# mclarsen/cuZFP

Measured on AMD Instinct MI355X. Metric: GB/s input encoded+decoded (device-resident), 3D f32 fixed-rate; % HBM peak, higher is better.
Workload: dtype f32; 1 GPU; 3d_float32_256^3_rate8; maxbits=512, parallelism=z-slab x1, stream_bytes_per_gpu=16777216

## Files before the change

cuzfp_amd/build.py:

```python
from __future__ import annotations

import os
import subprocess
import sys
from concurrent.futures import ThreadPoolExecutor

HERE = os.path.dirname(os.path.abspath(__file__))
ROOT = os.path.dirname(HERE)
CSRC = os.path.join(HERE, "csrc")
LIB = os.path.join(HERE, "lib")
BIN = os.path.join(HERE, "bin")
CLI = os.path.join(HERE, "cli")
OBJ = os.path.join(ROOT, "build", "obj")
INC = os.path.join(ROOT, "include")

ARCH = os.environ.get("CUZFP_OFFLOAD_ARCH", "gfx950")
HIPCC = os.environ.get("HIPCC", "/opt/rocm/bin/hipcc")
CXXFLAGS = ["-O3", "-std=c++17", "-fPIC", f"--offload-arch={ARCH}", f"-I{INC}",
            "-Wall", "-Wno-unused-function", "-Wno-pass-failed"]

KERNEL_UNITS = ["inst_f32", "inst_f64", "inst_i32", "inst_i64",
                "region_f32", "region_f64", "region_i32", "region_i64",
                "update_f32", "update_f64", "update_i32", "update_i64", "truncate",
                "variable_f32", "variable_f64", "region_variable_f32", "region_variable_f64", "truncate_variable",
                "region_variable_coarse_f32", "region_variable_coarse_f64",
                "region_variable_update_f32", "region_variable_update_f64",
                "region_variable_crop_f32", "region_variable_crop_f64",
                "capi"]
HEADERS = ["zfp_block.hpp", "kernels.hpp", "launch.hpp", "wave_index.hpp", "region.hpp", "region_kernels.hpp",
           "region_update_kernels.hpp", "rerate.hpp", "variable_kernels.hpp", "variable_index.hpp",
           "region_variable_kernels.hpp", "rerate_variable.hpp", "source_window.hpp", "variable_coarse.hpp",
           "region_variable_coarse_kernels.hpp", "region_variable_update_kernels.hpp",
           "region_variable_crop_kernels.hpp"]


def _newer(target: str, deps: list[str]) -> bool:
    if not os.path.exists(target):
        return True
    t = os.path.getmtime(target)
    return any(os.path.getmtime(d) > t for d in deps)


def _run(cmd: list[str]) -> None:
    r = subprocess.run(cmd, capture_output=True, text=True)
    if r.returncode != 0:
        sys.stderr.write(r.stdout + r.stderr)
        raise RuntimeError("build failed: " + " ".join(cmd))


def build(verbose: bool = False, jobs: int | None = None) -> dict:
    os.makedirs(LIB, exist_ok=True)
    os.makedirs(OBJ, exist_ok=True)
    hdrs = [os.path.join(CSRC, h) for h in HEADERS] + [os.path.join(INC, "cuzfp_hip.h")]
    jobs_list = []
    objs = []
    for u in KERNEL_UNITS:
        src = os.path.join(CSRC, u + ".hip")
        obj = os.path.join(OBJ, u + ".o")
        objs.append(obj)
        if _newer(obj, [src] + hdrs):
            jobs_list.append([HIPCC, *CXXFLAGS, "-c", src, "-o", obj])
    with ThreadPoolExecutor(max_workers=jobs or min(8, os.cpu_count() or 4)) as ex:
        for cmd in jobs_list:
            if verbose:
                print(" ".join(cmd))
        list(ex.map(_run, jobs_list))
    hip_so = os.path.join(LIB, "libcuzfp_hip.so")
    if jobs_list or _newer(hip_so, objs):
        _run([HIPCC, f"--offload-arch={ARCH}", "-shared", "-fPIC", "-o", hip_so, *objs])
    cpp_src = os.path.join(CSRC, "cuZFP.cpp")
    cpp_so = os.path.join(LIB, "libcuZFP.so")
    if _newer(cpp_so, [cpp_src, hip_so, os.path.join(INC, "cuZFP.h"),
                       os.path.join(INC, "zfp_structs.h")]):
        _run([HIPCC, "-O2", "-std=c++17", "-fPIC", "-shared", f"-I{INC}", "-o", cpp_so, cpp_src,
# ... 16 lines not shown
```

cuzfp_amd/csrc/kernels.hpp:

```cpp
#pragma once
#include <hip/hip_runtime.h>
#include <stdlib.h>

#include <atomic>
#include <type_traits>

#if defined(CUZFP_PROBE) && CUZFP_PROBE == 9
#define CUZFP_STAMP_WAVES 65536
__device__ uint64_t g_stamps[CUZFP_STAMP_WAVES * 10];
__device__ __forceinline__ uint32_t stamp_wave() { return blockIdx.x * (blockDim.x >> 6) + (threadIdx.x >> 6); }
#define ZFP_STAMP(i)                                                              \
  do {                                                                            \
    if ((threadIdx.x & 63) == 0 && stamp_wave() < CUZFP_STAMP_WAVES)              \
      g_stamps[stamp_wave() * 10 + 1 + (i)] = __builtin_amdgcn_s_memtime();      \
  } while (0)
__device__ __forceinline__ void stamp_hwid() {
  uint32_t hw, xcc;
  asm volatile("s_getreg_b32 %0, hwreg(HW_REG_HW_ID)" : "=s"(hw));
  asm volatile("s_getreg_b32 %0, hwreg(HW_REG_XCC_ID)" : "=s"(xcc));
  if ((threadIdx.x & 63) == 0 && stamp_wave() < CUZFP_STAMP_WAVES)
    g_stamps[stamp_wave() * 10] = (uint64_t)hw | ((uint64_t)xcc << 32);
}
__device__ __forceinline__ void stamp_real(int slot) {
  if ((threadIdx.x & 63) == 0 && stamp_wave() < CUZFP_STAMP_WAVES)
// ... 545 lines not shown
  asm volatile("s_waitcnt lgkmcnt(0)" ::: "memory");
  __builtin_amdgcn_wave_barrier();
}

template <int ROWS>
__device__ __forceinline__ void scatter_f64_staged(double* __restrict__ data, const Geometry& g, BlockPos bp,
                                                   const double* f, bool coded, uint64_t* wave_lds,
                                                   uint32_t lane) {
  static_assert(16 % ROWS == 0, "rows a pass");
  uint4* stage = (uint4*)wave_lds;
  double* base = data + ((size_t)(4 * bp.iz) * g.ny + 4 * bp.iy) * g.nx + 4 * (bp.ix - lane);
#pragma unroll
  for (int r0 = 0; r0 < 16; r0 += ROWS) {
    if (coded) {
#pragma unroll
      for (int j = 0; j < ROWS; j++) {
        uint4 a, b;
        __builtin_memcpy(&a, f + 4 * (r0 + j), 16);
        __builtin_memcpy(&b, f + 4 * (r0 + j) + 2, 16);
        stage[j * 128 + 2 * lane] = a;
        stage[j * 128 + 2 * lane + 1] = b;
      }
    } else {
#pragma unroll
      for (int j = 0; j < ROWS; j++) {
        stage[j * 128 + 2 * lane] = uint4{0, 0, 0, 0};
        stage[j * 128 + 2 * lane + 1] = uint4{0, 0, 0, 0};
      }
    }
    wave_lds_sync();
#pragma unroll
    for (int j = 0; j < ROWS; j++) {
      const int r = r0 + j, z = r >> 2, y = r & 3;
      double* row = base + ((size_t)z * g.ny + y) * g.nx;
      st16<true>(row + 2 * lane, stage[j * 128 + lane]);
      st16<true>(row + 128 + 2 * lane, stage[j * 128 + 64 + lane]);
    }
    if (r0 + ROWS < 16) wave_lds_sync();
  }
}

#ifndef CUZFP_F64_ENC_WAVES
#define CUZFP_F64_ENC_WAVES 2
#endif
#ifndef CUZFP_F64_DEC_WAVES
#define CUZFP_F64_DEC_WAVES 2
#endif
#ifndef CUZFP_F32_DEC_WAVES
#define CUZFP_F32_DEC_WAVES 4
#endif
#ifndef CUZFP_F32_ENC_WAVES
#define CUZFP_F32_ENC_WAVES 4
#endif
template <typename Scalar, int DIMS, bool ENC = false> struct occupancy {
  static constexpr int value = (sizeof(Scalar) == 8 && DIMS == 3) ? (ENC ? CUZFP_F64_ENC_WAVES : CUZFP_F64_DEC_WAVES)
                               : (sizeof(Scalar) == 4 && DIMS == 3) ? (ENC ? CUZFP_F32_ENC_WAVES : CUZFP_F32_DEC_WAVES)
                                                                    : 4;
};

template <typename Scalar, int DIMS, bool FAST, bool ALIGNED, bool PRIO = true, int REG = 0, int WPG = kEncWaves>
__device__ __forceinline__ void zfp_encode_body(const Scalar* __restrict__ data, const Geometry& g,
                                                uint64_t* __restrict__ stream, uint32_t bid,
                                                uint32_t* stab, uint32_t* ptab) {
  extern __shared__ __attribute__((aligned(16))) uint64_t lds_all[];
  constexpr int N = 1 << (2 * DIMS);
  const uint32_t wig = wave_in_group();
  const uint32_t wave = g.wave0 + bid * (blockDim.x >> 6) + wig;
  const uint32_t lane = threadIdx.x & 63;
  const uint32_t b = wave * kLanes + lane;
  const bool live_wave = wave < g.wave_end;
  uint64_t* lds = lds_all + (size_t)wig * g.lds_words;
  constexpr bool kGroupSpread = DIMS == 1 || REG != 0;
  if constexpr (DIMS == 2 && REG != 0) {
    for (uint32_t i = threadIdx.x; i < kSpreadTabBytes / 16; i += blockDim.x)
      ((uint4*)stab)[i] = ((const uint4*)g_spread_tab.e)[i];
    __syncthreads();
  }
  if constexpr (DIMS == 1) {
    if (threadIdx.x < 4) ((uint4*)stab)[threadIdx.x] = ((const uint4*)g_spread_tab.e)[threadIdx.x];
    for (uint32_t i = threadIdx.x; i < sizeof(Pair1dLut) / 16; i += blockDim.x)
      ((uint4*)ptab)[i] = ((const uint4*)g_pair1d_lut.e)[i];
    __syncthreads();
  }
  lds_spread* p1d = (lds_spread*)ptab;
  if (!live_wave) return;
  constexpr uint32_t kTabPieces = kSpreadTabBytes / 16;
  uint4 tab16[kTabPieces / kLanes];
  if constexpr (!kGroupSpread) {
#pragma unroll
    for (uint32_t i = 0; i < kTabPieces / kLanes; i++) tab16[i] = ((const uint4*)g_spread_tab.e)[lane + i * kLanes];
  }
  if constexpr (PRIO) __builtin_amdgcn_s_setprio(3);
  lds_spread* lut = (lds_spread*)stab;
  ZFP_STAMP_HWID();
  ZFP_STAMP_REAL(8);
  ZFP_STAMP(0);
  if constexpr (!ALIGNED) {
    for (uint32_t j = lane; j < g.maxbits + 2; j += kLanes) lds[j] = 0;
  }
  const uint32_t W = g.maxbits >> 6;
  Scalar f[N];
  if ((wave + 1) * kLanes <= g.nblocks) {
    gather<Scalar, DIMS, FAST>(data, g, block_pos<DIMS>(g, b), f);
  } else if (b < g.nblocks) {
    gather<Scalar, DIMS, FAST>(data, g, block_pos<DIMS>(g, b), f);
  } else if constexpr (ALIGNED && !REG) {
#pragma unroll
    for (int i = 0; i < N; i++) f[i] = (Scalar)0;
  }
  if constexpr (!kGroupSpread) {
#pragma unroll
    for (uint32_t i = 0; i < kTabPieces / kLanes; i++) ((uint4*)stab)[lane + i * kLanes] = tab16[i];
  }
  if constexpr (REG) {
    wave_lds_sync();
    uint64_t bits = 0;
    if (b < g.nblocks) {
      reg_writer<Scalar, PRIO, REG> wr{lut, p1d, 0, 0};
      if constexpr (REG == 2 || traits<Scalar>::is_int) wr.mb = g.maxbits;
      encode_block<Scalar, DIMS>(f, g.maxbits, wr);
      bits = wr.bits();
    }
    if constexpr (PRIO) __builtin_amdgcn_s_setprio(3);
    if constexpr (REG == 2) {
      if (b < g.nblocks) stream[b] = bits;
    } else {
      if (b < g.nblocks + (g.nblocks & 1u)) ((uint32_t*)stream)[b] = (uint32_t)bits;
    }
    return;
  }
  if constexpr (ALIGNED) {
    uint64_t* mine = lds + lane;
    for (uint32_t j = 0; j < W + kSlackWords; j++) mine[j * 64] = 0;
    if (g.wave0 + (bid + 1) * (blockDim.x >> 6) <= g.wave_end) {
      asm volatile("s_waitcnt vmcnt(0)" ::: "memory");
      __syncthreads();
    }
    wave_lds_sync();
    LdsOrWriter<PRIO> wr{mine, lut, 0, 64 * W, p1d, uniform_const64(0x7fffu)};
    encode_block<Scalar, DIMS>(f, g.maxbits, wr);
  } else if (b < g.nblocks) {
    {
      wave_lds_sync();
      LdsBitWriter<PRIO> wr{lds, lut, lane * g.maxbits, (lane + 1) * g.maxbits, 0, 0, p1d, uniform_const64(0x7fffu)};
      encode_block<Scalar, DIMS>(f, g.maxbits, wr);
    }
  }
  if constexpr (PRIO) __builtin_amdgcn_s_setprio(3);
  wave_lds_sync();
  const uint32_t nb = min((uint32_t)kLanes, g.nblocks - wave * kLanes);
  const uint32_t nwords = (nb * g.maxbits + 63) >> 6;
  uint64_t* out = stream + (size_t)wave * g.maxbits;
  if constexpr (ALIGNED) {
    if (nb == kLanes && g.vec_io && !(W & 1)) {
      uint32_t s, j, ds, dj;
      udivmod_uniform(2 * lane, W, s, j);
      udivmod_uniform(128u, W, ds, dj);
      for (uint32_t k = 2 * lane; k < kLanes * W; k += 128) {
        uint4 v;
        const uint64_t a0 = lds[j * 64 + s], a1 = lds[(j + 1) * 64 + s];
        __builtin_memcpy(&v.x, &a0, 8);
        __builtin_memcpy(&v.z, &a1, 8);
        st16<true>(&out[k], v);
        j += dj;
        s += ds;
        if (j >= W) { j -= W; s++; }
      }
      ZFP_STAMP(6);
      ZFP_STAMP_REAL(9);
      return;
    }
  }
  if constexpr (ALIGNED) {
    if (b < g.nblocks) {
      const uint64_t* mine = lds + lane;
      uint64_t* dst = out + (size_t)lane * W;
      if (g.vec_io && !(W & 1)) {
        for (uint32_t j = 0; j < W; j += 2) {
          uint4 v;
          const uint64_t a0 = mine[j * 64], a1 = mine[(j + 1) * 64];
          __builtin_memcpy(&v.x, &a0, 8);
          __builtin_memcpy(&v.z, &a1, 8);
          st16<kNtStream>(&dst[j], v);
        }
      } else {
        for (uint32_t j = 0; j < W; j++) dst[j] = mine[j * 64];
      }
    }
  } else if (g.vec_io) {
    const uint32_t npairs = nwords >> 1;
    for (uint32_t j = lane; j < npairs; j += kLanes)
      ((uint4*)out)[j] = ((const uint4*)lds)[j];
    if ((nwords & 1) && lane == 0) out[nwords - 1] = lds[nwords - 1];
  } else {
    for (uint32_t j = lane; j < nwords; j += kLanes) out[j] = lds[j];
  }
  ZFP_STAMP(6);
  ZFP_STAMP_REAL(9);
}

template <typename Scalar, int DIMS, bool FAST, bool ALIGNED, bool PRIO = true, int REG = 0, int WPG = kEncWaves>
__global__ __launch_bounds__(kLanes * WPG, (occupancy<Scalar, DIMS, true>::value)) void zfp_encode(const Scalar* __restrict__ data,
                                                                      Geometry g,
                                                                      uint64_t* __restrict__ stream) {
  __shared__ __attribute__((aligned(16))) uint32_t stab[512];
  __shared__ __attribute__((aligned(16))) uint32_t ptab[DIMS == 1 ? 1024 : 4];
  zfp_encode_body<Scalar, DIMS, FAST, ALIGNED, PRIO, REG, WPG>(data, g, stream, blockIdx.x, stab, ptab);
}

template <typename Scalar, int DIMS, bool FAST, bool PRIO = true, int REG = 0, int WPG = kDecWaves>
__device__ __forceinline__ void zfp_decode_body(const uint64_t* __restrict__ stream, const Geometry& g,
                                                Scalar* __restrict__ data, uint32_t bid,
                                                uint32_t* ctab, uint16_t* dtab) {
  extern __shared__ __attribute__((aligned(16))) uint64_t lds_all[];
  constexpr int N = 1 << (2 * DIMS);
  const uint32_t wig = wave_in_group();
  uint32_t wave;
  if constexpr (DIMS == 3 && !REG)
    wave = g.wave0 + decode_wave_of(bid, wig, blockDim.x >> 6, kEncWaves, g.xcd_remap != 0);
  else
    wave = g.wave0 + bid * (blockDim.x >> 6) + wig;
  const uint32_t lane = threadIdx.x & 63;
  const uint32_t b = wave * kLanes + lane;
  const bool live = wave < g.wave_end && b < g.nblocks;
  uint64_t* lds = lds_all + (size_t)wig * g.lds_words;
  uint32_t* lut = ctab;
  auto copy_dtab = [&]() {
    if constexpr (DIMS == 1)
      for (uint32_t i = threadIdx.x; i < sizeof(Plane1dDecLut) / 16; i += blockDim.x)
        ((uint4*)dtab)[i] = ((const uint4*)g_plane1d_lut.e)[i];
  };
  constexpr uint32_t kLutEnd = DIMS == 1 ? kLutPairs * 4 / 16 : sizeof(ChunkLut) / 16;
  const uint32_t* seg = (const uint32_t*)(stream + (size_t)wave * g.maxbits);
  uint32_t* L = (uint32_t*)lds + lane;
  uint64_t blk = 0;
  if constexpr (REG == 32) {
    if (live) blk = seg[lane];
    for (uint32_t i = threadIdx.x; i < kLutEnd; i += blockDim.x)
      ((uint4*)lut)[i] = ((const uint4*)g_chunk_lut.e)[i];
    copy_dtab();
  } else if constexpr (REG) {
    if (live) {
      const uint32_t nb = min((uint32_t)kLanes, g.nblocks - wave * kLanes);
      const uint32_t lim = ((nb * g.maxbits + 63) >> 6) * 2;
      const uint32_t s0 = lane * g.maxbits, d0 = s0 >> 5;
      const uint32_t a0 = seg[d0];
      const uint32_t a1 = d0 + 1 < lim ? seg[d0 + 1] : 0u;
      const uint32_t a2 = d0 + 2 < lim ? seg[d0 + 2] : 0u;
      blk = ((uint64_t)__builtin_amdgcn_alignbit(a1, a0, s0) |
             ((uint64_t)__builtin_amdgcn_alignbit(a2, a1, s0) << 32)) & lowmask(g.maxbits);
    }
    for (uint32_t i = threadIdx.x; i < kLutEnd; i += blockDim.x)
      ((uint4*)lut)[i] = ((const uint4*)g_chunk_lut.e)[i];
    copy_dtab();
  } else {
    const uint32_t D = (g.maxbits + 31) >> 5;
    const bool vec = (g.maxbits & 127) == 0 && g.vec_io;
    constexpr uint32_t kHeld = 8;
    uint4 held[kHeld];
    const bool cont = vec && wave < g.wave_end && g.nblocks - wave * kLanes >= kLanes && D <= 4 * kHeld;
    if (cont) {
      const uint4* src = (const uint4*)seg + lane;
#pragma unroll
      for (uint32_t q = 0; q < kHeld; q++)
        if (4 * q < D) held[q] = ld16<true>(&src[64 * q]);
    } else if (live && vec) {
      const uint4* src = (const uint4*)(seg + lane * D);
#pragma unroll
      for (uint32_t q = 0; q < kHeld; q++)
        if (4 * q < D) held[q] = ld16<kNtStream>(&src[q]);
    }
    for (uint32_t i = threadIdx.x; i < kLutEnd; i += blockDim.x)
      ((uint4*)lut)[i] = ((const uint4*)g_chunk_lut.e)[i];
    copy_dtab();
    if (cont) {
      uint32_t* L0 = (uint32_t*)lds;
      uint32_t sb, j, dsb, dj;
      udivmod_uniform(4 * lane, D, sb, j);
      udivmod_uniform(256u, D, dsb, dj);
#pragma unroll
      for (uint32_t q = 0; q < kHeld; q++)
        if (4 * q < D) {
          L0[(j) * 64 + sb] = held[q].x;
          L0[(j + 1) * 64 + sb] = held[q].y;
          L0[(j + 2) * 64 + sb] = held[q].z;
          L0[(j + 3) * 64 + sb] = held[q].w;
          j += dj;
          sb += dsb;
          if (j >= D) { j -= D; sb++; }
        }
    } else if (live) {
      if (vec) {
#pragma unroll
        for (uint32_t q = 0; q < kHeld; q++)
          if (4 * q < D) {
            L[(4 * q) * 64] = held[q].x;
            L[(4 * q + 1) * 64] = held[q].y;
            L[(4 * q + 2) * 64] = held[q].z;
            L[(4 * q + 3) * 64] = held[q].w;
          }
        const uint4* src = (const uint4*)(seg + lane * D);
        for (uint32_t q = 4 * kHeld; q < D; q += 4) {
          const uint4 v = src[q >> 2];
          L[q * 64] = v.x;
          L[(q + 1) * 64] = v.y;
          L[(q + 2) * 64] = v.z;
          L[(q + 3) * 64] = v.w;
        }
      } else {
        const uint32_t nb = min((uint32_t)kLanes, g.nblocks - wave * kLanes);
        const uint32_t lim = ((nb * g.maxbits + 63) >> 6) * 2;
        const uint32_t s0 = lane * g.maxbits, d0 = s0 >> 5;
        uint32_t prev = seg[d0];
        for (uint32_t j = 0; j < D; j++) {
          const uint32_t nxt = d0 + j + 1 < lim ? seg[d0 + j + 1] : 0u;
          L[j * 64] = __builtin_amdgcn_alignbit(nxt, prev, s0);
          prev = nxt;
        }
        if (g.maxbits & 31) L[(D - 1) * 64] &= (1u << (g.maxbits & 31)) - 1u;
      }
    } else if (wave < g.wave_end) {
      for (uint32_t j = 0; j < D; j++) L[j * 64] = 0;
    }
    if (wave < g.wave_end)
      for (uint32_t j = D; j < D + 5; j++) L[j * 64] = 0;
  }
  __syncthreads();
  if (wave >= g.wave_end) return;
  if constexpr (PRIO) __builtin_amdgcn_s_setprio(3);
  ZFP_STAMP_HWID();
  ZFP_STAMP_REAL(8);
  ZFP_STAMP(0);
  wave_lds_sync();
  ZFP_STAMP(5);
  {
    Scalar f[N];
    bool coded;
    if constexpr (REG) {
      RegReader<PRIO, REG == 32> rd;
      rd.lds32 = L;
      rd.lut32 = lut;
      rd.d1d = dtab;
      rd.set_block(blk);
      rd.init(0);
      coded = decode_block<Scalar, DIMS>(f, g.maxbits, rd);
    } else {
      LdsReader<PRIO> rd;
      rd.lds32 = L;
      rd.lut32 = lut;
      rd.d1d = dtab;
      rd.init(0);
      coded = decode_block<Scalar, DIMS>(f, g.maxbits, rd);
    }
    if constexpr (PRIO) __builtin_amdgcn_s_setprio(3);
    if constexpr (sizeof(Scalar) == 8 && DIMS == 3 && FAST && !REG) {
      if (g.row_stage) {
        const BlockPos bp = block_pos<DIMS>(g, b);
        if (g.row_stage == 4)
          scatter_f64_staged<4>((double*)data, g, bp, (const double*)f, coded, lds, lane);
        else if (g.row_stage == 2)
          scatter_f64_staged<2>((double*)data, g, bp, (const double*)f, coded, lds, lane);
        else
          scatter_f64_staged<1>((double*)data, g, bp, (const double*)f, coded, lds, lane);
        ZFP_STAMP(6);
        ZFP_STAMP_REAL(9);
        return;
      }
    }
    if (b < g.nblocks) {
      if (coded) {
        scatter<Scalar, DIMS, FAST>(data, g, block_pos<DIMS>(g, b), f);
      } else {
        Scalar z[N];
#pragma unroll
        for (int i = 0; i < N; i++) z[i] = (Scalar)0;
        scatter<Scalar, DIMS, FAST>(data, g, block_pos<DIMS>(g, b), z);
      }
    }
  }
  ZFP_STAMP(6);
  ZFP_STAMP_REAL(9);
}

template <typename Scalar, int DIMS, bool FAST, bool PRIO = true, int REG = 0, int WPG = kDecWaves>
__global__ __launch_bounds__(kLanes * WPG, (occupancy<Scalar, DIMS>::value)) void zfp_decode(const uint64_t* __restrict__ stream,
                                                                      Geometry g,
                                                                      Scalar* __restrict__ data) {
  __shared__ __attribute__((aligned(16))) uint32_t ctab[chunk_lut_bytes<DIMS>() / 4];
  __shared__ __attribute__((aligned(16))) uint16_t dtab[DIMS == 1 ? sizeof(Plane1dDecLut) / 2 : 8];
  zfp_decode_body<Scalar, DIMS, FAST, PRIO, REG, WPG>(stream, g, data, blockIdx.x, ctab, dtab);
}

template <typename Scalar, int DIMS, bool PRIO, int REG, int WPG, int K>
__global__ __launch_bounds__(kLanes * WPG, (occupancy<Scalar, DIMS, true>::value)) void zfp_encode_regk(
    const Scalar* __restrict__ data, Geometry g, uint64_t* __restrict__ stream) {
  static_assert(DIMS <= 2 && (REG == 1 || REG == 2) && K >= 2 && K <= 8, "register-writer batches: 1D/2D");
  constexpr int N = 1 << (2 * DIMS);
  __shared__ __attribute__((aligned(16))) uint32_t stab[512];
  __shared__ __attribute__((aligned(16))) uint32_t ptab[DIMS == 1 ? 1024 : 4];
  const uint32_t wig = wave_in_group();
  const uint32_t lane = threadIdx.x & 63;
  const uint32_t w0 = g.wave0 + (blockIdx.x * WPG + wig) * K;
  Scalar f[K][N];
#pragma unroll
  for (int k = 0; k < K; k++) {
    const uint32_t b = (w0 + k) * kLanes + lane;
    if (w0 + k < g.wave_end && b < g.nblocks) gather<Scalar, DIMS, true>(data, g, block_pos<DIMS>(g, b), f[k]);
  }
  if constexpr (DIMS == 2) {
    for (uint32_t i = threadIdx.x; i < kSpreadTabBytes / 16; i += blockDim.x)
      ((uint4*)stab)[i] = ((const uint4*)g_spread_tab.e)[i];
  } else {
    if (threadIdx.x < 4) ((uint4*)stab)[threadIdx.x] = ((const uint4*)g_spread_tab.e)[threadIdx.x];
    for (uint32_t i = threadIdx.x; i < sizeof(Pair1dLut) / 16; i += blockDim.x)
      ((uint4*)ptab)[i] = ((const uint4*)g_pair1d_lut.e)[i];
  }
  __syncthreads();
  lds_spread* lut = (lds_spread*)stab;
  lds_spread* p1d = (lds_spread*)ptab;
#pragma unroll
  for (int k = 0; k < K; k++) {
    const uint32_t b = (w0 + k) * kLanes + lane;
    if (w0 + k >= g.wave_end) break;
    uint64_t bits = 0;
    if (b < g.nblocks) {
      if constexpr (PRIO) __builtin_amdgcn_s_setprio(3);
      reg_writer<Scalar, PRIO, REG> wr{lut, p1d, 0, 0};
      if constexpr (REG == 2 || traits<Scalar>::is_int) wr.mb = g.maxbits;
      encode_block<Scalar, DIMS>(f[k], g.maxbits, wr);
      bits = wr.bits();
    }
    if constexpr (REG == 2) {
      if (b < g.nblocks) stream[b] = bits;
    } else {
      if (b < g.nblocks + (g.nblocks & 1u)) ((uint32_t*)stream)[b] = (uint32_t)bits;
    }
  }
}

__device__ __forceinline__ uint64_t reg_block(const uint64_t* stream, const Geometry& g, uint32_t wave,
                                              uint32_t lane) {
  const uint32_t* seg = (const uint32_t*)(stream + (size_t)wave * g.maxbits);
  const uint32_t nb = min((uint32_t)kLanes, g.nblocks - wave * kLanes);
// ... 63 lines not shown
  static const long forced = [] {
    const char* e = getenv("CUZFP_LDS_CAP_BYTES");
    return (e && *e) ? atol(e) : 0L;
  }();
  if (forced > 0) return (size_t)forced;
  static std::atomic<int> cap[kMaxDevices];
  int dev = 0;
  if (hipGetDevice(&dev) != hipSuccess || dev < 0 || dev >= kMaxDevices) return 65536;
  int c = cap[dev].load(std::memory_order_relaxed);
  if (!c) {
    int n = 0;
    if (hipDeviceGetAttribute(&n, hipDeviceAttributeMaxSharedMemoryPerBlock, dev) != hipSuccess || n <= 0)
      n = 65536;
    cap[dev].store(n, std::memory_order_relaxed);
    c = n;
  }
  return (size_t)c;
}

static inline uint32_t waves_per_group(uint32_t lds_words, size_t shared_bytes, uint32_t most) {
  const size_t cap = lds_cap_bytes();
  uint32_t w = most;
  while (w > 1 && (size_t)w * lds_words * 8 + shared_bytes > cap) w >>= 1;
  return w;
}

static inline bool within_rounds(uint32_t nwaves, int waves_per_simd, uint32_t rounds) {
  static std::atomic<int> cus[kMaxDevices];
  int dev = 0, c = 256;
  if (hipGetDevice(&dev) == hipSuccess && dev >= 0 && dev < kMaxDevices) {
    c = cus[dev].load(std::memory_order_relaxed);
    if (!c) {
      int n = 0;
      if (hipDeviceGetAttribute(&n, hipDeviceAttributeMultiprocessorCount, dev) != hipSuccess || n <= 0) n = 256;
      cus[dev].store(n, std::memory_order_relaxed);
      c = n;
    }
  }
  return nwaves <= (uint32_t)c * 4u * (uint32_t)waves_per_simd * rounds;
}
static inline bool use_priority(uint32_t nwaves, int waves_per_simd, uint32_t rounds) {
  static const int forced = [] {
    const char* e = getenv("CUZFP_PRIO");
    return (e && *e) ? (atoi(e) != 0 ? 1 : 0) : -1;
  }();
  if (forced >= 0) return forced != 0;
  return within_rounds(nwaves, waves_per_simd, rounds);
}

#if defined(CUZFP_XVAR)
constexpr bool kFastOnly = true;
#else
constexpr bool kFastOnly = false;
#endif
#ifndef CUZFP_ENC_PRIO_ROUNDS
#define CUZFP_ENC_PRIO_ROUNDS 1
#endif
template <typename Scalar, int DIMS>
int launch_encode_t(const void* data, const Geometry& g, bool fast, uint64_t* stream,
                           uint32_t wave0, uint32_t nwaves, hipStream_t st) {
  Geometry gg = g;
  gg.wave0 = wave0;
  gg.wave_end = wave0 + nwaves;
  gg.vec_io = (g.maxbits % 2 == 0) && ((uintptr_t)stream % 16 == 0);
  gg.lds_words = g.maxbits + kLanes * kSlackWords;
  constexpr size_t kStatic = kSpreadTabBytes + (DIMS == 1 ? sizeof(Pair1dLut) : 16);
  const Scalar* d = (const Scalar*)data;
  if constexpr (DIMS <= 2) {
    if (g.maxbits == 32 || g.maxbits == 64) {
      gg.lds_words = 0;
      const dim3 grid((nwaves + kWavesPerGroup - 1) / kWavesPerGroup), block(kLanes * kWavesPerGroup);
      const bool prio = use_priority(nwaves, occupancy<Scalar, DIMS, true>::value, CUZFP_ENC_PRIO_ROUNDS);
#define ZFP_ENC_REG(FAST_, PRIO_)                                                                          \
  do {                                                                                                     \
    if (g.maxbits == 64)                                                                                   \
      hipLaunchKernelGGL((zfp_encode<Scalar, DIMS, FAST_, true, PRIO_, 2, kWavesPerGroup>), grid, block, 0, st, d, gg, stream); \
    else                                                                                                   \
      hipLaunchKernelGGL((zfp_encode<Scalar, DIMS, FAST_, true, PRIO_, 1, kWavesPerGroup>), grid, block, 0, st, d, gg, stream); \
  } while (0)
      if constexpr (DIMS == 1 && kRegEncBatch1d > 1) {
        if (fast && nwaves >= kRegBatchMinWaves) {
          constexpr int W = kWavesPerGroup, K = kRegEncBatch1d;
          const uint32_t phys = (nwaves + K - 1) / K;
          const dim3 kgrid((phys + W - 1) / W), kblock(kLanes * W);
          if (g.maxbits == 64)
            hipLaunchKernelGGL((zfp_encode_regk<Scalar, DIMS, false, 2, W, K>), kgrid, kblock, 0, st, d, gg, stream);
          else
            hipLaunchKernelGGL((zfp_encode_regk<Scalar, DIMS, false, 1, W, K>), kgrid, kblock, 0, st, d, gg, stream);
          const hipError_t e = hipGetLastError();
          t_last_hip = e;
          return e == hipSuccess ? CUZFP_SUCCESS : CUZFP_ERROR_HIP;
        }
      }
      if (fast && prio) ZFP_ENC_REG(true, true);
      else if (fast) ZFP_ENC_REG(true, false);
      else if (prio) ZFP_ENC_REG(false, true);
      else ZFP_ENC_REG(false, false);
#undef ZFP_ENC_REG
      const hipError_t e = hipGetLastError();
      t_last_hip = e;
      return e == hipSuccess ? CUZFP_SUCCESS : CUZFP_ERROR_HIP;
    }
  }
  const bool aligned = (g.maxbits & 63) == 0 && gg.lds_words * 8 + kStatic <= lds_cap_bytes();
  if (!aligned) gg.lds_words = g.maxbits + 2;
  gg.row_stage = 0;
  if (gg.lds_words * 8 + kStatic > lds_cap_bytes()) return CUZFP_ERROR_INVALID_ARGUMENT;
  const uint32_t wpg = waves_per_group(gg.lds_words, kStatic, kEncWaves);
  const dim3 grid((nwaves + wpg - 1) / wpg), block(kLanes * wpg);
  const size_t lds = (size_t)wpg * gg.lds_words * 8;
  if (fast && aligned && !use_priority(nwaves, occupancy<Scalar, DIMS, true>::value, CUZFP_ENC_PRIO_ROUNDS))
    hipLaunchKernelGGL((zfp_encode<Scalar, DIMS, true, true, false>), grid, block, lds, st, d, gg, stream);
  else if (fast && aligned)
    hipLaunchKernelGGL((zfp_encode<Scalar, DIMS, true, true>), grid, block, lds, st, d, gg, stream);
  else if (fast)
    hipLaunchKernelGGL((zfp_encode<Scalar, DIMS, true, false>), grid, block, lds, st, d, gg, stream);
  else if constexpr (kFastOnly)
    return CUZFP_ERROR_UNSUPPORTED_TYPE;
  else if (aligned)
    hipLaunchKernelGGL((zfp_encode<Scalar, DIMS, false, true>), grid, block, lds, st, d, gg, stream);
  else
    hipLaunchKernelGGL((zfp_encode<Scalar, DIMS, false, false>), grid, block, lds, st, d, gg, stream);
  const hipError_t e = hipGetLastError();
  t_last_hip = e;
  return e == hipSuccess ? CUZFP_SUCCESS : CUZFP_ERROR_HIP;
}

template <typename Scalar, int DIMS>
int launch_decode_t(const uint64_t* stream, const Geometry& g, bool fast, void* data,
                           uint32_t wave0, uint32_t nwaves, hipStream_t st) {
  Geometry gg = g;
  gg.wave0 = wave0;
  gg.wave_end = wave0 + nwaves;
  gg.vec_io = (g.maxbits % 2 == 0) && ((uintptr_t)stream % 16 == 0);
  gg.lds_words = ((g.maxbits + 31) / 32 + 5) * 32;
  gg.row_stage = 0;
  if (sizeof(Scalar) == 8 && DIMS == 3 && fast && g.bx % kLanes == 0) {
    const size_t img = (size_t)gg.lds_words * 8;
    gg.row_stage = img >= 4 * 2048 ? 4 : img >= 2 * 2048 ? 2 : img >= 2048 ? 1 : 0;
  }
  const bool reg = DIMS <= 2 && g.maxbits <= 64;
  if (reg) gg.lds_words = 0;
  const size_t kStatic = chunk_lut_bytes<DIMS>() + (DIMS == 1 ? sizeof(Plane1dDecLut) : 16);
  if (gg.lds_words * 8 + kStatic > lds_cap_bytes()) return CUZFP_ERROR_INVALID_ARGUMENT;
  const uint32_t wpg = waves_per_group(gg.lds_words, kStatic, kDecWaves);
  const dim3 grid((nwaves + wpg - 1) / wpg), block(kLanes * wpg);
  const size_t lds = (size_t)wpg * gg.lds_words * 8;
  Scalar* d = (Scalar*)data;
  if constexpr (DIMS <= 2) {
    if (reg) {
      const bool prio = use_priority(nwaves, occupancy<Scalar, DIMS>::value, 2);
      if constexpr (DIMS == 1 && kRegDecBatch1d > 1) {
        if (fast && nwaves >= kRegBatchMinWaves) {
          constexpr int W = kRegBatchWaves1d, K = kRegDecBatch1d;
          const uint32_t phys = (nwaves + K - 1) / K;
          const dim3 kgrid((phys + W - 1) / W), kblock(kLanes * W);
          constexpr bool P = CUZFP_REG_BATCH_PRIO;
          if (g.maxbits == 32)
            hipLaunchKernelGGL((zfp_decode_regk<Scalar, DIMS, true, P, W, K, 32>), kgrid, kblock, 0, st, stream, gg, d);
          else
            hipLaunchKernelGGL((zfp_decode_regk<Scalar, DIMS, true, P, W, K, 64>), kgrid, kblock, 0, st, stream, gg, d);
          const hipError_t e = hipGetLastError();
          t_last_hip = e;
          return e == hipSuccess ? CUZFP_SUCCESS : CUZFP_ERROR_HIP;
        }
      }
      constexpr int W = DIMS == 1 ? kRegWaves1d : kRegWaves2d;
      const dim3 rgrid((nwaves + W - 1) / W), rblock(kLanes * W);
      auto go = [&](auto rb) {
        constexpr int RB = decltype(rb)::value;
        if (fast && prio)
          hipLaunchKernelGGL((zfp_decode<Scalar, DIMS, true, true, RB, W>), rgrid, rblock, 0, st, stream, gg, d);
        else if (fast)
          hipLaunchKernelGGL((zfp_decode<Scalar, DIMS, true, false, RB, W>), rgrid, rblock, 0, st, stream, gg, d);
        else if (prio)
          hipLaunchKernelGGL((zfp_decode<Scalar, DIMS, false, true, RB, W>), rgrid, rblock, 0, st, stream, gg, d);
        else
          hipLaunchKernelGGL((zfp_decode<Scalar, DIMS, false, false, RB, W>), rgrid, rblock, 0, st, stream, gg, d);
      };
      if (g.maxbits == 32)
        go(std::integral_constant<int, 32>{});
      else
        go(std::integral_constant<int, 64>{});
      const hipError_t e = hipGetLastError();
      t_last_hip = e;
      return e == hipSuccess ? CUZFP_SUCCESS : CUZFP_ERROR_HIP;
    }
  }
  constexpr uint32_t kDecPrioRounds = (sizeof(Scalar) == 8 && DIMS == 3) ? 1 : 2;
  if constexpr (DIMS == 3 && sizeof(Scalar) == 4 && kDecWavesRound > kDecWaves) {
    constexpr uint32_t R = kDecWavesRound;
    if (within_rounds(nwaves, occupancy<Scalar, DIMS>::value, 1) && decode_remap_ok(nwaves, R, kEncWaves) &&
        (size_t)R * gg.lds_words * 8 + kStatic <= lds_cap_bytes() &&
        waves_per_group(g.maxbits + kLanes * kSlackWords, kSpreadTabBytes + 16, kEncWaves) == (uint32_t)kEncWaves &&
        use_priority(nwaves, occupancy<Scalar, DIMS>::value, kDecPrioRounds)) {
      gg.xcd_remap = 1;
      const dim3 rgrid(nwaves / R), rblock(kLanes * R);
      const size_t rlds = (size_t)R * gg.lds_words * 8;
      if (fast)
        hipLaunchKernelGGL((zfp_decode<Scalar, DIMS, true, true, 0, R>), rgrid, rblock, rlds, st, stream, gg, d);
      else if constexpr (!kFastOnly)
        hipLaunchKernelGGL((zfp_decode<Scalar, DIMS, false, true, 0, R>), rgrid, rblock, rlds, st, stream, gg, d);
      else
        return CUZFP_ERROR_UNSUPPORTED_TYPE;
      const hipError_t e = hipGetLastError();
      t_last_hip = e;
      return e == hipSuccess ? CUZFP_SUCCESS : CUZFP_ERROR_HIP;
    }
  }
  if (fast && !use_priority(nwaves, occupancy<Scalar, DIMS>::value, kDecPrioRounds))
    hipLaunchKernelGGL((zfp_decode<Scalar, DIMS, true, false>), grid, block, lds, st, stream, gg, d);
  else if (fast)
    hipLaunchKernelGGL((zfp_decode<Scalar, DIMS, true>), grid, block, lds, st, stream, gg, d);
  else if constexpr (!kFastOnly)
    hipLaunchKernelGGL((zfp_decode<Scalar, DIMS, false>), grid, block, lds, st, stream, gg, d);
  const hipError_t e = hipGetLastError();
  t_last_hip = e;
  return e == hipSuccess ? CUZFP_SUCCESS : CUZFP_ERROR_HIP;
}


#if defined(CUZFP_XVAR)
#include "../../tools/xvar_launch.hpp"
#else
template <typename Scalar>
int launch_encode_type(const Problem& p, const void* data, bool fast, uint64_t* stream,
                       uint32_t wave0, uint32_t nwaves, hipStream_t st) {
  switch (p.dims) {
    case 1: return launch_encode_t<Scalar, 1>(data, p.g, fast, stream, wave0, nwaves, st);
    case 2: return launch_encode_t<Scalar, 2>(data, p.g, fast, stream, wave0, nwaves, st);
    default: return launch_encode_t<Scalar, 3>(data, p.g, fast, stream, wave0, nwaves, st);
  }
}

template <typename Scalar>
int launch_decode_type(const Problem& p, const uint64_t* stream, bool fast, void* data,
                       uint32_t wave0, uint32_t nwaves, hipStream_t st) {
  switch (p.dims) {
    case 1: return launch_decode_t<Scalar, 1>(stream, p.g, fast, data, wave0, nwaves, st);
    case 2: return launch_decode_t<Scalar, 2>(stream, p.g, fast, data, wave0, nwaves, st);
    default: return launch_decode_t<Scalar, 3>(stream, p.g, fast, data, wave0, nwaves, st);
  }
}

#endif

}
```

cuzfp_amd/csrc/launch.hpp:

```cpp
#pragma once
#include <hip/hip_runtime.h>
#include <stdint.h>

#include "../../include/cuzfp_hip.h"
#include "region.hpp"

namespace cuzfp {

constexpr int kLanes = 64;
constexpr int kMaxDevices = 64;

struct Geometry {
  uint32_t nx, ny, nz;
  uint32_t bx, by;
  uint32_t nblocks;
  uint32_t maxbits;
  uint32_t wave0;
  uint32_t wave_end;
  uint32_t vec_io;
  uint32_t lds_words;
  int64_t sx, sy, sz;
  uint32_t dbx_m, dbx_s, dpl_m, dpl_s, divmagic;
  uint32_t row_stage;
  uint32_t xcd_remap;
};

inline void set_divisor(uint32_t d, uint32_t& m, uint32_t& s) {
  uint32_t l = 0;
  while ((1ull << l) < d) l++;
  s = 31 + l;
  m = (uint32_t)(((1ull << s) + d - 1) / d);
}

inline Region make_region(const Geometry& g, uint32_t ox, uint32_t oy, uint32_t oz, uint32_t ex,
                          uint32_t ey, uint32_t ez, int64_t sx, int64_t sy, int64_t sz) {
  Region r;
  r.bx = g.bx;
  r.by = g.by;
  r.bx0 = ox / 4;
  r.by0 = oy / 4;
  r.bz0 = oz / 4;
  r.rbx = (uint32_t)(((uint64_t)ox + ex + 3) / 4) - r.bx0;
  r.rby = (uint32_t)(((uint64_t)oy + ey + 3) / 4) - r.by0;
  r.rbz = (uint32_t)(((uint64_t)oz + ez + 3) / 4) - r.bz0;
  const uint64_t n = (uint64_t)r.rbx * r.rby * r.rbz;
  r.nrb = (uint32_t)n;
  r.ox = ox; r.oy = oy; r.oz = oz;
  r.ex = ex; r.ey = ey; r.ez = ez;
  r.maxbits = g.maxbits;
  set_divisor(r.rbx, r.drx_m, r.drx_s);
  set_divisor(r.rbx * r.rby, r.drp_m, r.drp_s);
  r.divmagic = n < (1ull << 31) ? 1u : 0u;
  r.stream_dwords = (((uint64_t)g.nblocks * g.maxbits + 63) / 64) * 2;
  r.sx = sx ? sx : 1;
  r.sy = sy ? sy : (int64_t)ex;
  r.sz = sz ? sz : (int64_t)ex * ey;
  return r;
}

struct Problem {
  int type;
  unsigned dims;
  Geometry g;
  bool fast_ok;
};

extern thread_local int t_last_hip;

template <typename Scalar>
int launch_encode_type(const Problem& p, const void* data, bool fast, uint64_t* stream,
                       uint32_t wave0, uint32_t nwaves, hipStream_t st);
template <typename Scalar>
int launch_decode_type(const Problem& p, const uint64_t* stream, bool fast, void* data,
                       uint32_t wave0, uint32_t nwaves, hipStream_t st);
template <typename Scalar>
int launch_decode_region_type(const Problem& p, const Region& r, const uint64_t* stream, bool fast,
                              uint32_t budget, void* out, hipStream_t st);

inline bool region_covered(const Geometry& g, const Region& r) {
  auto axis = [](uint32_t o, uint32_t e, uint32_t n) { return !(o & 3) && (!((o + e) & 3) || o + e == n); };
  return axis(r.ox, r.ex, g.nx) && axis(r.oy, r.ey, g.ny) && axis(r.oz, r.ez, g.nz);
}

template <typename Scalar>
// ... 58 lines not shown
```

Before: 1451 GB/s.

## Specialize 3D f32 encode/decode kernels on compile-time block word count

Adds template-specialized encode and decode kernels for 3D float with maxbits of 256, 512 or 1024, instantiated in separate compilation units and selected at launch. With the block size known at compile time, LDS zeroing loops are unrolled, the udivmod-based transposes between LDS and global memory become fixed strided copies, and the spread table is loaded once cooperatively per group instead of once per wave. The aim is to cut integer address arithmetic, loop overhead and redundant table loads on the hot path. The cost is more kernel variants and a larger binary, plus possible changes in register pressure.

```diff
diff --git a/cuzfp_amd/build.py b/cuzfp_amd/build.py
--- a/cuzfp_amd/build.py
+++ b/cuzfp_amd/build.py
@@ -20,6 +20,7 @@
             "-Wall", "-Wno-unused-function", "-Wno-pass-failed"]
 
 KERNEL_UNITS = ["inst_f32", "inst_f64", "inst_i32", "inst_i64",
+                "inst_f32_w4", "inst_f32_w8", "inst_f32_w16",
                 "region_f32", "region_f64", "region_i32", "region_i64",
                 "update_f32", "update_f64", "update_i32", "update_i64", "truncate",
                 "variable_f32", "variable_f64", "region_variable_f32", "region_variable_f64", "truncate_variable",
diff --git a/cuzfp_amd/csrc/inst_f32_w16.hip b/cuzfp_amd/csrc/inst_f32_w16.hip
--- /dev/null
+++ b/cuzfp_amd/csrc/inst_f32_w16.hip
@@ -0,0 +1,11 @@
+#if !defined(CUZFP_XVAR)
+#define CUZFP_SIZED_UNIT
+#include "kernels.hpp"
+
+namespace cuzfp {
+template void launch_encode_sized<float, 16>(const float*, const Geometry&, uint64_t*, dim3, dim3, size_t, bool,
+                                          hipStream_t);
+template void launch_decode_sized<float, 16>(const uint64_t*, const Geometry&, float*, dim3, dim3, size_t, int,
+                                          hipStream_t);
+}
+#endif
diff --git a/cuzfp_amd/csrc/inst_f32_w4.hip b/cuzfp_amd/csrc/inst_f32_w4.hip
--- /dev/null
+++ b/cuzfp_amd/csrc/inst_f32_w4.hip
@@ -0,0 +1,11 @@
+#if !defined(CUZFP_XVAR)
+#define CUZFP_SIZED_UNIT
+#include "kernels.hpp"
+
+namespace cuzfp {
+template void launch_encode_sized<float, 4>(const float*, const Geometry&, uint64_t*, dim3, dim3, size_t, bool,
+                                          hipStream_t);
+template void launch_decode_sized<float, 4>(const uint64_t*, const Geometry&, float*, dim3, dim3, size_t, int,
+                                          hipStream_t);
+}
+#endif
diff --git a/cuzfp_amd/csrc/inst_f32_w8.hip b/cuzfp_amd/csrc/inst_f32_w8.hip
--- /dev/null
+++ b/cuzfp_amd/csrc/inst_f32_w8.hip
@@ -0,0 +1,11 @@
+#if !defined(CUZFP_XVAR)
+#define CUZFP_SIZED_UNIT
+#include "kernels.hpp"
+
+namespace cuzfp {
+template void launch_encode_sized<float, 8>(const float*, const Geometry&, uint64_t*, dim3, dim3, size_t, bool,
+                                          hipStream_t);
+template void launch_decode_sized<float, 8>(const uint64_t*, const Geometry&, float*, dim3, dim3, size_t, int,
+                                          hipStream_t);
+}
+#endif
diff --git a/cuzfp_amd/csrc/kernels.hpp b/cuzfp_amd/csrc/kernels.hpp
--- a/cuzfp_amd/csrc/kernels.hpp
+++ b/cuzfp_amd/csrc/kernels.hpp
@@ -621,13 +621,22 @@
 #ifndef CUZFP_F32_ENC_WAVES
 #define CUZFP_F32_ENC_WAVES 4
 #endif
+#ifndef CUZFP_ENC_FULL_START
+#define CUZFP_ENC_FULL_START 1
+#endif
+#ifndef CUZFP_ENC_GROUP_TABLES
+#define CUZFP_ENC_GROUP_TABLES 1
+#endif
+constexpr bool kEncFullStart = CUZFP_ENC_FULL_START != 0;
+constexpr bool kEncGroupTables = CUZFP_ENC_GROUP_TABLES != 0;
 template <typename Scalar, int DIMS, bool ENC = false> struct occupancy {
   static constexpr int value = (sizeof(Scalar) == 8 && DIMS == 3) ? (ENC ? CUZFP_F64_ENC_WAVES : CUZFP_F64_DEC_WAVES)
                                : (sizeof(Scalar) == 4 && DIMS == 3) ? (ENC ? CUZFP_F32_ENC_WAVES : CUZFP_F32_DEC_WAVES)
                                                                     : 4;
 };
 
-template <typename Scalar, int DIMS, bool FAST, bool ALIGNED, bool PRIO = true, int REG = 0, int WPG = kEncWaves>
+template <typename Scalar, int DIMS, bool FAST, bool ALIGNED, bool PRIO = true, int REG = 0, int WPG = kEncWaves,
+          int BW = 0>
 __device__ __forceinline__ void zfp_encode_body(const Scalar* __restrict__ data, const Geometry& g,
                                                 uint64_t* __restrict__ stream, uint32_t bid,
                                                 uint32_t* stab, uint32_t* ptab) {
@@ -638,7 +647,10 @@
   const uint32_t lane = threadIdx.x & 63;
   const uint32_t b = wave * kLanes + lane;
   const bool live_wave = wave < g.wave_end;
-  uint64_t* lds = lds_all + (size_t)wig * g.lds_words;
+  static_assert(BW == 0 || (ALIGNED && !REG && DIMS == 3 && (BW == 4 || BW == 8 || BW == 16)), "block_words");
+  const uint32_t maxbits = BW ? 64u * BW : g.maxbits;
+  const uint32_t lds_words = BW ? 64u * BW + kLanes * kSlackWords : g.lds_words;
+  uint64_t* lds = lds_all + (size_t)wig * lds_words;
   constexpr bool kGroupSpread = DIMS == 1 || REG != 0;
   if constexpr (DIMS == 2 && REG != 0) {
     for (uint32_t i = threadIdx.x; i < kSpreadTabBytes / 16; i += blockDim.x)
@@ -654,8 +666,16 @@
   lds_spread* p1d = (lds_spread*)ptab;
   if (!live_wave) return;
   constexpr uint32_t kTabPieces = kSpreadTabBytes / 16;
+  const bool group_tabs = BW != 0 && kEncGroupTables && g.wave0 + (bid + 1) * (blockDim.x >> 6) <= g.wave_end;
+  static_assert(kTabPieces == 2 * kLanes, "two pieces a lane");
   uint4 tab16[kTabPieces / kLanes];
-  if constexpr (!kGroupSpread) {
+  uint4 tab_a = {0, 0, 0, 0}, tab_b = {0, 0, 0, 0};
+  const uint32_t piece_a = group_tabs ? threadIdx.x : lane;
+  const uint32_t piece_b = group_tabs ? threadIdx.x + blockDim.x : lane + kLanes;
+  if constexpr (BW != 0) {
+    if (piece_a < kTabPieces) tab_a = ((const uint4*)g_spread_tab.e)[piece_a];
+    if (piece_b < kTabPieces) tab_b = ((const uint4*)g_spread_tab.e)[piece_b];
+  } else if constexpr (!kGroupSpread) {
 #pragma unroll
     for (uint32_t i = 0; i < kTabPieces / kLanes; i++) tab16[i] = ((const uint4*)g_spread_tab.e)[lane + i * kLanes];
   }
@@ -667,9 +687,12 @@
   if constexpr (!ALIGNED) {
     for (uint32_t j = lane; j < g.maxbits + 2; j += kLanes) lds[j] = 0;
   }
-  const uint32_t W = g.maxbits >> 6;
+  const uint32_t W = maxbits >> 6;
   Scalar f[N];
-  if ((wave + 1) * kLanes <= g.nblocks) {
+  if (BW != 0 && kEncFullStart && (wave + 1) * kLanes <= g.nblocks) {
+    gather<Scalar, DIMS, FAST>(data, g, block_pos<DIMS>(g, b), f);
+    asm volatile("; a wave of live blocks");
+  } else if ((wave + 1) * kLanes <= g.nblocks) {
     gather<Scalar, DIMS, FAST>(data, g, block_pos<DIMS>(g, b), f);
   } else if (b < g.nblocks) {
     gather<Scalar, DIMS, FAST>(data, g, block_pos<DIMS>(g, b), f);
@@ -677,7 +700,10 @@
 #pragma unroll
     for (int i = 0; i < N; i++) f[i] = (Scalar)0;
   }
-  if constexpr (!kGroupSpread) {
+  if constexpr (BW != 0) {
+    if (piece_a < kTabPieces) ((uint4*)stab)[piece_a] = tab_a;
+    if (piece_b < kTabPieces) ((uint4*)stab)[piece_b] = tab_b;
+  } else if constexpr (!kGroupSpread) {
 #pragma unroll
     for (uint32_t i = 0; i < kTabPieces / kLanes; i++) ((uint4*)stab)[lane + i * kLanes] = tab16[i];
   }
@@ -700,14 +726,19 @@
   }
   if constexpr (ALIGNED) {
     uint64_t* mine = lds + lane;
-    for (uint32_t j = 0; j < W + kSlackWords; j++) mine[j * 64] = 0;
+    if constexpr (BW != 0) {
+#pragma unroll
+      for (uint32_t j = 0; j < BW + kSlackWords; j++) mine[j * 64] = 0;
+    } else {
+      for (uint32_t j = 0; j < W + kSlackWords; j++) mine[j * 64] = 0;
+    }
     if (g.wave0 + (bid + 1) * (blockDim.x >> 6) <= g.wave_end) {
       asm volatile("s_waitcnt vmcnt(0)" ::: "memory");
       __syncthreads();
     }
     wave_lds_sync();
     LdsOrWriter<PRIO> wr{mine, lut, 0, 64 * W, p1d, uniform_const64(0x7fffu)};
-    encode_block<Scalar, DIMS>(f, g.maxbits, wr);
+    encode_block<Scalar, DIMS>(f, maxbits, wr);
   } else if (b < g.nblocks) {
     {
       wave_lds_sync();
@@ -718,9 +749,25 @@
   if constexpr (PRIO) __builtin_amdgcn_s_setprio(3);
   wave_lds_sync();
   const uint32_t nb = min((uint32_t)kLanes, g.nblocks - wave * kLanes);
-  const uint32_t nwords = (nb * g.maxbits + 63) >> 6;
-  uint64_t* out = stream + (size_t)wave * g.maxbits;
-  if constexpr (ALIGNED) {
+  const uint32_t nwords = (nb * maxbits + 63) >> 6;
+  uint64_t* out = stream + (size_t)wave * maxbits;
+  if constexpr (BW != 0) {
+    if (nb == kLanes) {
+      static_assert(128 % BW == 0 && BW % 2 == 0, "block_words");
+      const uint64_t* src = lds + ((2 * lane) % BW) * 64 + (2 * lane) / BW;
+#pragma unroll
+      for (uint32_t t = 0; t < BW / 2; t++) {
+        uint4 v;
+        const uint64_t a0 = src[t * (128 / BW)], a1 = src[64 + t * (128 / BW)];
+        __builtin_memcpy(&v.x, &a0, 8);
+        __builtin_memcpy(&v.z, &a1, 8);
+        st16<true>(&out[2 * lane + 128 * t], v);
+      }
+      ZFP_STAMP(6);
+      ZFP_STAMP_REAL(9);
+      return;
+    }
+  } else if constexpr (ALIGNED) {
     if (nb == kLanes && g.vec_io && !(W & 1)) {
       uint32_t s, j, ds, dj;
       udivmod_uniform(2 * lane, W, s, j);
@@ -768,16 +815,17 @@
   ZFP_STAMP_REAL(9);
 }
 
-template <typename Scalar, int DIMS, bool FAST, bool ALIGNED, bool PRIO = true, int REG = 0, int WPG = kEncWaves>
+template <typename Scalar, int DIMS, bool FAST, bool ALIGNED, bool PRIO = true, int REG = 0, int WPG = kEncWaves,
+          int BW = 0>
 __global__ __launch_bounds__(kLanes * WPG, (occupancy<Scalar, DIMS, true>::value)) void zfp_encode(const Scalar* __restrict__ data,
                                                                       Geometry g,
                                                                       uint64_t* __restrict__ stream) {
   __shared__ __attribute__((aligned(16))) uint32_t stab[512];
   __shared__ __attribute__((aligned(16))) uint32_t ptab[DIMS == 1 ? 1024 : 4];
-  zfp_encode_body<Scalar, DIMS, FAST, ALIGNED, PRIO, REG, WPG>(data, g, stream, blockIdx.x, stab, ptab);
-}
-
-template <typename Scalar, int DIMS, bool FAST, bool PRIO = true, int REG = 0, int WPG = kDecWaves>
+  zfp_encode_body<Scalar, DIMS, FAST, ALIGNED, PRIO, REG, WPG, BW>(data, g, stream, blockIdx.x, stab, ptab);
+}
+
+template <typename Scalar, int DIMS, bool FAST, bool PRIO = true, int REG = 0, int WPG = kDecWaves, int BW = 0>
 __device__ __forceinline__ void zfp_decode_body(const uint64_t* __restrict__ stream, const Geometry& g,
                                                 Scalar* __restrict__ data, uint32_t bid,
                                                 uint32_t* ctab, uint16_t* dtab) {
@@ -792,7 +840,10 @@
   const uint32_t lane = threadIdx.x & 63;
   const uint32_t b = wave * kLanes + lane;
   const bool live = wave < g.wave_end && b < g.nblocks;
-  uint64_t* lds = lds_all + (size_t)wig * g.lds_words;
+  static_assert(BW == 0 || (!REG && DIMS == 3 && (BW == 4 || BW == 8 || BW == 16)), "block_words");
+  const uint32_t maxbits = BW ? 64u * BW : g.maxbits;
+  const uint32_t lds_words = BW ? (2u * BW + 5) * 32 : g.lds_words;
+  uint64_t* lds = lds_all + (size_t)wig * lds_words;
   uint32_t* lut = ctab;
   auto copy_dtab = [&]() {
     if constexpr (DIMS == 1)
@@ -800,7 +851,7 @@
         ((uint4*)dtab)[i] = ((const uint4*)g_plane1d_lut.e)[i];
   };
   constexpr uint32_t kLutEnd = DIMS == 1 ? kLutPairs * 4 / 16 : sizeof(ChunkLut) / 16;
-  const uint32_t* seg = (const uint32_t*)(stream + (size_t)wave * g.maxbits);
+  const uint32_t* seg = (const uint32_t*)(stream + (size_t)wave * maxbits);
   uint32_t* L = (uint32_t*)lds + lane;
   uint64_t blk = 0;
   if constexpr (REG == 32) {
@@ -823,8 +874,8 @@
       ((uint4*)lut)[i] = ((const uint4*)g_chunk_lut.e)[i];
     copy_dtab();
   } else {
-    const uint32_t D = (g.maxbits + 31) >> 5;
-    const bool vec = (g.maxbits & 127) == 0 && g.vec_io;
+    const uint32_t D = (maxbits + 31) >> 5;
+    const bool vec = BW != 0 || ((maxbits & 127) == 0 && g.vec_io);
     constexpr uint32_t kHeld = 8;
     uint4 held[kHeld];
     const bool cont = vec && wave < g.wave_end && g.nblocks - wave * kLanes >= kLanes && D <= 4 * kHeld;
@@ -844,6 +895,18 @@
     copy_dtab();
     if (cont) {
       uint32_t* L0 = (uint32_t*)lds;
+      if constexpr (BW != 0) {
+        constexpr uint32_t DW = 2 * BW;
+        static_assert(256 % DW == 0 && DW % 4 == 0 && DW <= 4 * kHeld, "block_words");
+        uint32_t* dst = L0 + ((4 * lane) % DW) * 64 + (4 * lane) / DW;
+#pragma unroll
+        for (uint32_t q = 0; q < DW / 4; q++) {
+          dst[q * (256 / DW)] = held[q].x;
+          dst[64 + q * (256 / DW)] = held[q].y;
+          dst[128 + q * (256 / DW)] = held[q].z;
+          dst[192 + q * (256 / DW)] = held[q].w;
+        }
+      } else {
       uint32_t sb, j, dsb, dj;
       udivmod_uniform(4 * lane, D, sb, j);
       udivmod_uniform(256u, D, dsb, dj);
@@ -858,6 +921,7 @@
           sb += dsb;
           if (j >= D) { j -= D; sb++; }
         }
+      }
     } else if (live) {
       if (vec) {
 #pragma unroll
@@ -891,8 +955,14 @@
     } else if (wave < g.wave_end) {
       for (uint32_t j = 0; j < D; j++) L[j * 64] = 0;
     }
-    if (wave < g.wave_end)
-      for (uint32_t j = D; j < D + 5; j++) L[j * 64] = 0;
+    if (wave < g.wave_end) {
+      if constexpr (BW != 0) {
+#pragma unroll
+        for (uint32_t j = 2 * BW; j < 2 * BW + 5; j++) L[j * 64] = 0;
+      } else {
+        for (uint32_t j = D; j < D + 5; j++) L[j * 64] = 0;
+      }
+    }
   }
   __syncthreads();
   if (wave >= g.wave_end) return;
@@ -919,7 +989,7 @@
       rd.lut32 = lut;
       rd.d1d = dtab;
       rd.init(0);
-      coded = decode_block<Scalar, DIMS>(f, g.maxbits, rd);
+      coded = decode_block<Scalar, DIMS>(f, maxbits, rd);
     }
     if constexpr (PRIO) __builtin_amdgcn_s_setprio(3);
     if constexpr (sizeof(Scalar) == 8 && DIMS == 3 && FAST && !REG) {
@@ -951,13 +1021,13 @@
   ZFP_STAMP_REAL(9);
 }
 
-template <typename Scalar, int DIMS, bool FAST, bool PRIO = true, int REG = 0, int WPG = kDecWaves>
+template <typename Scalar, int DIMS, bool FAST, bool PRIO = true, int REG = 0, int WPG = kDecWaves, int BW = 0>
 __global__ __launch_bounds__(kLanes * WPG, (occupancy<Scalar, DIMS>::value)) void zfp_decode(const uint64_t* __restrict__ stream,
                                                                       Geometry g,
                                                                       Scalar* __restrict__ data) {
   __shared__ __attribute__((aligned(16))) uint32_t ctab[chunk_lut_bytes<DIMS>() / 4];
   __shared__ __attribute__((aligned(16))) uint16_t dtab[DIMS == 1 ? sizeof(Plane1dDecLut) / 2 : 8];
-  zfp_decode_body<Scalar, DIMS, FAST, PRIO, REG, WPG>(stream, g, data, blockIdx.x, ctab, dtab);
+  zfp_decode_body<Scalar, DIMS, FAST, PRIO, REG, WPG, BW>(stream, g, data, blockIdx.x, ctab, dtab);
 }
 
 template <typename Scalar, int DIMS, bool PRIO, int REG, int WPG, int K>
@@ -1127,6 +1197,37 @@
 constexpr bool kFastOnly = true;
 #else
 constexpr bool kFastOnly = false;
+#endif
+#ifndef CUZFP_BLOCK_WORDS
+#define CUZFP_BLOCK_WORDS 1
+#endif
+constexpr bool kBlockWords = CUZFP_BLOCK_WORDS != 0;
+template <typename Scalar, int BW>
+void launch_encode_sized(const Scalar* d, const Geometry& gg, uint64_t* stream, dim3 grid, dim3 block, size_t lds,
+                         bool prio, hipStream_t st);
+template <typename Scalar, int BW>
+void launch_decode_sized(const uint64_t* stream, const Geometry& gg, Scalar* d, dim3 grid, dim3 block, size_t lds,
+                         int form, hipStream_t st);
+#if defined(CUZFP_SIZED_UNIT) || defined(CUZFP_XVAR)
+template <typename Scalar, int BW>
+void launch_encode_sized(const Scalar* d, const Geometry& gg, uint64_t* stream, dim3 grid, dim3 block, size_t lds,
+                         bool prio, hipStream_t st) {
+  if (prio)
+    hipLaunchKernelGGL((zfp_encode<Scalar, 3, true, true, true, 0, kEncWaves, BW>), grid, block, lds, st, d, gg, stream);
+  else
+    hipLaunchKernelGGL((zfp_encode<Scalar, 3, true, true, false, 0, kEncWaves, BW>), grid, block, lds, st, d, gg, stream);
+}
+template <typename Scalar, int BW>
+void launch_decode_sized(const uint64_t* stream, const Geometry& gg, Scalar* d, dim3 grid, dim3 block, size_t lds,
+                         int form, hipStream_t st) {
+  constexpr int R = kDecWavesRound > kDecWaves ? kDecWavesRound : kDecWaves;
+  if (form == 2 && R > kDecWaves)
+    hipLaunchKernelGGL((zfp_decode<Scalar, 3, true, true, 0, R, BW>), grid, block, lds, st, stream, gg, d);
+  else if (form != 0)
+    hipLaunchKernelGGL((zfp_decode<Scalar, 3, true, true, 0, kDecWaves, BW>), grid, block, lds, st, stream, gg, d);
+  else
+    hipLaunchKernelGGL((zfp_decode<Scalar, 3, true, false, 0, kDecWaves, BW>), grid, block, lds, st, stream, gg, d);
+}
 #endif
 #ifndef CUZFP_ENC_PRIO_ROUNDS
 #define CUZFP_ENC_PRIO_ROUNDS 1
@@ -1184,6 +1285,18 @@
   const uint32_t wpg = waves_per_group(gg.lds_words, kStatic, kEncWaves);
   const dim3 grid((nwaves + wpg - 1) / wpg), block(kLanes * wpg);
   const size_t lds = (size_t)wpg * gg.lds_words * 8;
+  if constexpr (DIMS == 3 && std::is_same<Scalar, float>::value && kBlockWords) {
+    const int bw = block_words(sizeof(Scalar), DIMS, fast, aligned, gg.vec_io != 0, g.maxbits);
+    if (bw) {
+      const bool prio = use_priority(nwaves, occupancy<Scalar, DIMS, true>::value, CUZFP_ENC_PRIO_ROUNDS);
+      if (bw == 4) launch_encode_sized<Scalar, 4>(d, gg, stream, grid, block, lds, prio, st);
+      else if (bw == 8) launch_encode_sized<Scalar, 8>(d, gg, stream, grid, block, lds, prio, st);
+      else launch_encode_sized<Scalar, 16>(d, gg, stream, grid, block, lds, prio, st);
+      const hipError_t e = hipGetLastError();
+      t_last_hip = e;
+      return e == hipSuccess ? CUZFP_SUCCESS : CUZFP_ERROR_HIP;
+    }
+  }
   if (fast && aligned && !use_priority(nwaves, occupancy<Scalar, DIMS, true>::value, CUZFP_ENC_PRIO_ROUNDS))
     hipLaunchKernelGGL((zfp_encode<Scalar, DIMS, true, true, false>), grid, block, lds, st, d, gg, stream);
   else if (fast && aligned)
@@ -1263,6 +1376,17 @@
     }
   }
   constexpr uint32_t kDecPrioRounds = (sizeof(Scalar) == 8 && DIMS == 3) ? 1 : 2;
+  int bw = 0;
+  if constexpr (DIMS == 3 && std::is_same<Scalar, float>::value && kBlockWords)
+    bw = block_words(sizeof(Scalar), DIMS, fast, true, gg.vec_io != 0, g.maxbits);
+  auto sized = [&](int form, const dim3& gr, const dim3& bl, size_t bytes) {
+    if constexpr (DIMS == 3 && std::is_same<Scalar, float>::value && kBlockWords) {
+      if (bw == 4) launch_decode_sized<Scalar, 4>(stream, gg, d, gr, bl, bytes, form, st);
+      else if (bw == 8) launch_decode_sized<Scalar, 8>(stream, gg, d, gr, bl, bytes, form, st);
+      else if (bw == 16) launch_decode_sized<Scalar, 16>(stream, gg, d, gr, bl, bytes, form, st);
+    }
+    return bw != 0;
+  };
   if constexpr (DIMS == 3 && sizeof(Scalar) == 4 && kDecWavesRound > kDecWaves) {
     constexpr uint32_t R = kDecWavesRound;
     if (within_rounds(nwaves, occupancy<Scalar, DIMS>::value, 1) && decode_remap_ok(nwaves, R, kEncWaves) &&
@@ -1272,7 +1396,8 @@
       gg.xcd_remap = 1;
       const dim3 rgrid(nwaves / R), rblock(kLanes * R);
       const size_t rlds = (size_t)R * gg.lds_words * 8;
-      if (fast)
+      if (sized(2, rgrid, rblock, rlds)) {
+      } else if (fast)
         hipLaunchKernelGGL((zfp_decode<Scalar, DIMS, true, true, 0, R>), rgrid, rblock, rlds, st, stream, gg, d);
       else if constexpr (!kFastOnly)
         hipLaunchKernelGGL((zfp_decode<Scalar, DIMS, false, true, 0, R>), rgrid, rblock, rlds, st, stream, gg, d);
@@ -1283,7 +1408,9 @@
       return e == hipSuccess ? CUZFP_SUCCESS : CUZFP_ERROR_HIP;
     }
   }
-  if (fast && !use_priority(nwaves, occupancy<Scalar, DIMS>::value, kDecPrioRounds))
+  if (bw) {
+    sized(use_priority(nwaves, occupancy<Scalar, DIMS>::value, kDecPrioRounds) ? 1 : 0, grid, block, lds);
+  } else if (fast && !use_priority(nwaves, occupancy<Scalar, DIMS>::value, kDecPrioRounds))
     hipLaunchKernelGGL((zfp_decode<Scalar, DIMS, true, false>), grid, block, lds, st, stream, gg, d);
   else if (fast)
     hipLaunchKernelGGL((zfp_decode<Scalar, DIMS, true>), grid, block, lds, st, stream, gg, d);
diff --git a/cuzfp_amd/csrc/launch.hpp b/cuzfp_amd/csrc/launch.hpp
--- a/cuzfp_amd/csrc/launch.hpp
+++ b/cuzfp_amd/csrc/launch.hpp
@@ -30,6 +30,11 @@
   while ((1ull << l) < d) l++;
   s = 31 + l;
   m = (uint32_t)(((1ull << s) + d - 1) / d);
+}
+
+inline int block_words(size_t scalar_bytes, unsigned dims, bool fast, bool aligned, bool vec_io, uint32_t maxbits) {
+  if (scalar_bytes != 4 || dims != 3 || !fast || !aligned || !vec_io) return 0;
+  return maxbits == 256 ? 4 : maxbits == 512 ? 8 : maxbits == 1024 ? 16 : 0;
 }
 
 inline Region make_region(const Geometry& g, uint32_t ox, uint32_t oy, uint32_t oz, uint32_t ex,
```

Result: no change. 1449 GB/s (-0.1%).
